# 011235813/cm3

Measured on AMD Instinct MI355X. Metric: env-steps/s (all agents, whole node), higher is better.
Workload: dtype f32; 1 GPU; config_particle_stage2_antipodal.json: 4 agents, 4096 vectorised envs per GPU, max_steps=33, auto-reset, trajectory mode (every tick writes slot t+1 of a [330+1, E, ...] device trajectory incl. termin; envs_per_gpu=4096, n_agents=4, global_envs=4096, mode=trajectory, live_state=True, ticks_per_launch=1, parallelism=env-sharded x1, no data-path collective

## Files before the change

### cm3_amd/csrc/particle.hip

```cpp
#include "common.h"
#include "philox.h"
#include "thresholds.h"

#ifdef CM3_PARTICLE_ILP_TU
#define CM3_PARTICLE_TU 1
#else
#define CM3_PARTICLE_TU 0
#endif

namespace cm3 {

struct ParticleParams;
int particle_ilp_launch_pairs_f32(const ParticleParams &p, int n_agents, int waves_per_wg, hipStream_t stream);
int particle_ilp_launch_agents_f32(const ParticleParams &p, int n_agents, int waves_per_wg, hipStream_t stream);
[[maybe_unused]] constexpr size_t kIlpMaxWaves = 16384;

struct ParticleParams {
  int E;
  int max_steps;
  uint32_t flags;
  int _pad;
  int E0, EN;
  int64_t env_id_base;
  uint64_t seed;
// ... 418 lines not shown
#pragma unroll 1
  for (int t = 0; t < n_ticks; ++t) {
    int act[N];
    int32_t *actions_t = tick_ptr(p.actions, p.st_actions, t);
    if (gen) {
#pragma unroll
      for (int i = 0; i < N; ++i) act[i] = rand5(action_word(ablock[i], episode, (uint32_t)steps));
      if (active) store_row<int32_t, N>(actions_t, e, act);
    } else {
      load_row<int32_t, N>(actions_t, ec, act);
    }

    R fx[N], fy[N];
#pragma unroll
    for (int i = 0; i < N; ++i) {
      R ux = R(0), uy = R(0);
      if (act[i] == 1) ux = R(-1);
      if (act[i] == 2) ux = R(+1);
      if (act[i] == 3) uy = R(-1);
      if (act[i] == 4) uy = R(+1);
      fx[i] = ux * R(5.0) + R(0.0);
      fy[i] = uy * R(5.0) + R(0.0);
    }

#pragma unroll
    for (int a = 0; a < N; ++a) {
#pragma unroll
      for (int b = a + 1; b < N; ++b) {
        R f_x, f_y;
        contact_force<R>(s[a].z - s[b].z, s[a].w - s[b].w, f_x, f_y);
        fx[a] = f_x + fx[a];
        fy[a] = f_y + fy[a];
        fx[b] = (-f_x) + fx[b];
        fy[b] = (-f_y) + fy[b];
      }
    }

#pragma unroll
    for (int i = 0; i < N; ++i) {
      s[i].x = s[i].x * kKeep;
      s[i].y = s[i].y * kKeep;
      s[i].x = s[i].x + (fx[i] / R(1.0)) * kDt;
      s[i].y = s[i].y + (fy[i] / R(1.0)) * kDt;
      s[i].z = s[i].z + s[i].x * kDt;
      s[i].w = s[i].w + s[i].y * kDt;
    }
    steps += 1;
    CM3_STAMP(2, false);

    R rew[N];
    bool all_reached = true;
#pragma unroll
    for (int i = 0; i < N; ++i) {
      const R dx = s[i].z - g[i].x, dy = s[i].w - g[i].y;
      const R d2 = dx * dx + dy * dy;
      rew[i] = R(0) - Math<R>::sqrt(d2);
      all_reached = all_reached && (d2 < Thresh<R>::kReach2);
    }
#pragma unroll
    for (int a = 0; a < N; ++a) {
#pragma unroll
      for (int b = a + 1; b < N; ++b) {
        if (is_collision<R>(s[b].z - s[a].z, s[b].w - s[a].w)) {
          rew[a] = rew[a] - R(1);
          rew[b] = rew[b] - R(1);
          collisions += 2;
        }
      }
    }
    const R reward = sum_agents<R, N>(rew);
    const bool done = (steps == p.max_steps) || all_reached;

    CM3_STAMP(3, false);
    if (active) {
      store_row<R, N>(reinterpret_cast<R *>(tick_ptr(p.reward_n, p.st_reward_n, t)), e, rew);
      reinterpret_cast<R *>(tick_ptr(p.reward, p.st_reward, t))[e] = reward;
      tick_ptr(p.done, p.st_done, t)[e] = done ? 1 : 0;
      if (p.collisions_tick) tick_ptr(p.collisions_tick, p.st_coll, t)[e] = collisions;
    }
    CM3_STAMP(8, false);

    bool was_reset = false;
    if (auto_reset && done) {
      if (active) {
        void *term_state = tick_ptr(p.term_state, p.st_term_state, t);
        void *term_obs = tick_ptr(p.term_obs_others, p.st_term_obs, t);
        if (term_state) {
          V4 *t4 = reinterpret_cast<V4 *>(term_state);
#pragma unroll
          for (int i = 0; i < N; ++i) t4[(size_t)i * E + e] = s[i];
        }
        if (term_obs) store_obs_others_direct<R, N>(s, e, reinterpret_cast<R *>(term_obs));
      }
      episode += 1;
      init_episode<R, N, true>(p, genv, episode, s, g, preset_table(0));
      steps = 0;
      collisions = 0;
      was_reset = true;
    }
    CM3_STAMP(9, false);

    if (active) {
      V4 *sout4 = reinterpret_cast<V4 *>(tick_ptr(p.state_out, p.st_state, t));
#pragma unroll
      for (int i = 0; i < N; ++i) sout4[(size_t)i * E + e] = s[i];
      if (p.goals_out != p.goals_in || was_reset) {
        V2 *gout2 = reinterpret_cast<V2 *>(tick_ptr(p.goals_out, p.st_goals, t));
#pragma unroll
        for (int i = 0; i < N; ++i) gout2[(size_t)i * E + e] = g[i];
      }
      if (p.state_copy) {
#pragma unroll
        for (int i = 0; i < N; ++i) store_obs_vec<SP>(reinterpret_cast<V4 *>(p.state_copy) + ((size_t)i * E + e), s[i]);
      }
      if (was_reset && p.goals_copy) {
#pragma unroll
        for (int i = 0; i < N; ++i) reinterpret_cast<V2 *>(p.goals_copy)[(size_t)i * E + e] = g[i];
      }
    }

    CM3_STAMP(4, false);
    store_obs_others_staged<R, N, SP>(s, &lds_all[wave][0], lane, e0, p.EN,
                                      reinterpret_cast<R *>(tick_ptr(p.obs_others, p.st_obs, t)));
    CM3_STAMP(5, false);
  }

  if (active) {
    int2 m;
    m.x = steps;
    m.y = collisions;
    reinterpret_cast<int2 *>(p.meta_out)[e] = m;
    if (episode != episode_in) p.episode[e] = (int32_t)episode;
  }
  CM3_STAMP(6, true);
  CM3_SPAN_OUT(p.span);
}




template <int N> struct PairGeom {
  static constexpr int NO = N - 1;
  static constexpr int SLOTS = N * NO;
  static constexpr int LA = (N >= 3 && N <= 5) ? (N == 3 ? 2 : 4) : NO;
  static constexpr int pow2ceil(int v) {
    int r = 1;
    while (r < v) r <<= 1;
    return r;
  }
  static constexpr int G = pow2ceil(N * LA);
  static constexpr int EPW = 64 / G;
};

template <typename R, int N, int WAVES, bool FUSED, int SP = kSpPlain, bool LIVE = false, int TU = CM3_PARTICLE_TU>
__global__ void __launch_bounds__(WAVES * 64)
    k_particle_step_pairs(const void *h_state_in, const void *h_goals_in, const int32_t *h_meta_in, const int32_t *h_episode,
                          const int h_E, const uint32_t h_flags, const int h_E0, const int h_EN, const int h_max_steps,
                          const int32_t *h_actions, const ParticleParams p) {
  static_assert(N >= 2, "the pair mapping needs at least two agents");
  using V4 = typename Vec<R>::v4;
  using V2 = typename Vec<R>::v2;
  using PG = PairGeom<N>;
  constexpr int NO = PG::NO, SLOTS = PG::SLOTS, G = PG::G, EPW = PG::EPW, LA = PG::LA;
  static_assert(PairGeom<N>::pow2ceil(SLOTS) == G, "the padded lane layout must not change the group size");
  CM3_SPAN_IN();

  const int lane = threadIdx.x & 63, wave_all = threadIdx.x >> 6;
  const int wave = wave_all;
  const int gslot = lane & (G - 1), sub = lane / G, base = lane - gslot;
  const uint32_t E = (uint32_t)h_E, EN = (uint32_t)h_EN;
  const uint32_t e = (uint32_t)h_E0 + (cm3_xcd_block(h_flags) * WAVES + wave) * EPW + sub;
  const bool env_ok = e < EN;
  const uint32_t ec = env_ok ? e : EN - 1;
  const int i_raw = gslot / LA, k_raw = gslot - i_raw * LA;
  const bool slot_ok = i_raw < N && k_raw < NO;
  const int i = slot_ok ? i_raw : 0, k = slot_ok ? k_raw : 0, j = k < i ? k : k + 1;
  const int vslot = i * NO + k;
  const bool lead = slot_ok && k == 0;
  const bool head = gslot == 0;

  CM3_STAMP(0, false);
  const uint32_t row_i = (uint32_t)i * E, row_j = (uint32_t)j * E;
  V4 si = *at32<const V4>(h_state_in, (row_i + ec) * (uint32_t)sizeof(V4));
  V4 sj = *at32<const V4>(h_state_in, (row_j + ec) * (uint32_t)sizeof(V4));
  V2 gl = *at32<const V2>(h_goals_in, (row_i + ec) * (uint32_t)sizeof(V2));
  const int2 meta = *at32<const int2>(h_meta_in, ec * 8u);
  int steps = meta.x, collisions = meta.y;
  const bool auto_reset = (h_flags & CM3_FLAG_AUTO_RESET) != 0;
  const bool gen = (h_flags & CM3_FLAG_GEN_ACTIONS) != 0;
  uint32_t episode = 0;
  if (gen || (h_flags & CM3_FLAG_AUTO_RESET)) episode = (uint32_t)*at32<const int32_t>(h_episode, ec * 4u);
  const uint32_t episode_in = episode;
  CM3_FETCH_EARLY(p.state_out, p.goals_out, p.goals_in, p.collisions_tick, p.reward_n, p.reward, p.done, p.obs_others, p.meta_out);
  if constexpr (LIVE) CM3_FETCH_EARLY(p.state_copy, p.goals_copy);
  const uint64_t genv = (uint64_t)(p.env_id_base + (int64_t)ec);
  uint32_t aword = 0;
  if (gen) aword = pick_word(action_block(p.seed, genv, (uint32_t)(i >> 2)), i & 3);
  const R kDt = R(0.1), kKeep = R(1 - 0.25);

  CM3_STAMP(1, true);
  CM3_SPAN_MARK(0, true);
  const int n_ticks = FUSED ? p.n_ticks : 1;
#pragma unroll 1
  for (int t = 0; t < n_ticks; ++t) {
    int32_t *actions_t = tick_ptr(p.actions, p.st_actions, t);
    int act = 0;
    R f_x, f_y;
    if (gen) {
      act = rand5(action_word(aword, episode, (uint32_t)steps));
    } else {
      act = *at32<const int32_t>(actions_t, (ec * N + i) * 4u);
    }

    CM3_STAMP(2, false);
    CM3_SPAN_MARK(1, false);
    R ux = R(0), uy = R(0);
    if (act == 1) ux = R(-1);
    if (act == 2) ux = R(+1);
    if (act == 3) uy = R(-1);
    if (act == 4) uy = R(+1);
    R Fx = ux * R(5.0) + R(0.0), Fy = uy * R(5.0) + R(0.0);
    contact_force<R>(si.z - sj.z, si.w - sj.w, f_x, f_y);
    CM3_STAMP(3, false);
    if constexpr (sizeof(R) == 4 && LA == 4 && NO >= 3) {
      Fx = dpp_f32<0x00>(f_x) + Fx;
      Fy = dpp_f32<0x00>(f_y) + Fy;
      Fx = dpp_f32<0x55>(f_x) + Fx;
      Fy = dpp_f32<0x55>(f_y) + Fy;
      Fx = dpp_f32<0xAA>(f_x) + Fx;
      Fy = dpp_f32<0xAA>(f_y) + Fy;
      if constexpr (NO == 4) {
        Fx = dpp_f32<0xFF>(f_x) + Fx;
        Fy = dpp_f32<0xFF>(f_y) + Fy;
      }
    } else if constexpr (N == 2) {
      Fx = f_x + Fx;
      Fy = f_y + Fy;
    } else if constexpr (sizeof(R) == 4 && LA == 2) {
      Fx = dpp_f32<0xA0>(f_x) + Fx;
      Fy = dpp_f32<0xA0>(f_y) + Fy;
      Fx = dpp_f32<0xF5>(f_x) + Fx;
      Fy = dpp_f32<0xF5>(f_y) + Fy;
    } else {
#pragma unroll
      for (int kk = 0; kk < NO; ++kk) {
        const int src = base + i * LA + kk;
        Fx = __shfl(f_x, src, 64) + Fx;
        Fy = __shfl(f_y, src, 64) + Fy;
      }
    }

    si.x = si.x * kKeep;
    si.y = si.y * kKeep;
    si.x = si.x + (Fx / R(1.0)) * kDt;
    si.y = si.y + (Fy / R(1.0)) * kDt;
    si.z = si.z + si.x * kDt;
    si.w = si.w + si.y * kDt;
    steps += 1;
    if constexpr (N == 2 && sizeof(R) == 4) {
      sj.x = dpp_f32<kDppXor1>(si.x);
      sj.y = dpp_f32<kDppXor1>(si.y);
      sj.z = dpp_f32<kDppXor1>(si.z);
      sj.w = dpp_f32<kDppXor1>(si.w);
    } else {
      const int src = base + j * LA;
      sj.x = __shfl(si.x, src, 64);
      sj.y = __shfl(si.y, src, 64);
      sj.z = __shfl(si.z, src, 64);
      sj.w = __shfl(si.w, src, 64);
    }

    CM3_STAMP(4, true);
    CM3_SPAN_MARK(2, false);
    R rew;
    bool reached;
    {
      const R dx = si.z - gl.x, dy = si.w - gl.y;
      const R d2 = dx * dx + dy * dy;
      rew = R(0) - Math<R>::sqrt(d2);
      reached = d2 < Thresh<R>::kReach2;
    }
    const bool hit = slot_ok && is_collision<R>(sj.z - si.z, sj.w - si.w);
    const unsigned long long hits = __ballot(hit);
    const unsigned long long grp = (G == 64) ? hits : ((hits >> base) & ((1ull << (G & 63)) - 1ull));
    const int c_i = __popcll((grp >> (i * LA)) & ((1ull << NO) - 1ull));
#pragma unroll
    for (int c = 0; c < NO; ++c)
      if (c < c_i) rew = rew - R(1);
    collisions += __popcll(grp);
    const unsigned long long rb = __ballot(reached && lead);
    const unsigned long long rgrp = (G == 64) ? rb : ((rb >> base) & ((1ull << (G & 63)) - 1ull));
    const bool all_reached = __popcll(rgrp) == N;
    R rews[N];
    if constexpr (N == 2 && sizeof(R) == 4) {
      rews[0] = dpp_f32<0xA0>(rew);
      rews[1] = dpp_f32<0xF5>(rew);
    } else if constexpr (N == 4 && sizeof(R) == 4) {
      rews[0] = dpp_f32<kDppBcast + 0 * LA>(rew);
      rews[1] = dpp_f32<kDppBcast + 1 * LA>(rew);
      rews[2] = dpp_f32<kDppBcast + 2 * LA>(rew);
      rews[3] = dpp_f32<kDppBcast + 3 * LA>(rew);
    } else {
#pragma unroll
      for (int a = 0; a < N; ++a) rews[a] = __shfl(rew, base + a * LA, 64);
    }
    const R reward = sum_agents<R, N>(rews);
    const bool done = (steps == h_max_steps) || all_reached;

    const int collisions_tick = collisions;

    CM3_STAMP(5, true);
    CM3_SPAN_MARK(3, false);
    bool was_reset = false;
    if (auto_reset && done) {
      if (env_ok) {
        void *term_state = tick_ptr(p.term_state, p.st_term_state, t);
        void *term_obs = tick_ptr(p.term_obs_others, p.st_term_obs, t);
        if (term_state && lead) *at32<V4>(term_state, (row_i + e) * (uint32_t)sizeof(V4)) = si;
        if (term_obs && slot_ok) *at32<V4>(term_obs, (e * SLOTS + vslot) * (uint32_t)sizeof(V4)) = sub4<R, V4>(sj, si);
      }
      episode += 1;
      const uint64_t rseed = reset_seed(p);
      const bool rnd = episode_is_random(p, genv, episode, rseed);
      V2 gj;
      init_agent<R, N, true>(p, genv, episode, rnd, i, si, gl, preset_table(), &rseed);
      init_agent<R, N, true>(p, genv, episode, rnd, j, sj, gj, preset_table(), &rseed);
      steps = 0;
      collisions = 0;
      was_reset = true;
    }

    CM3_STAMP(6, false);
    if (env_ok) {
      if (lead) {
        if (gen) *at32<int32_t>(actions_t, (e * N + i) * 4u) = act;
        *at32<R>(tick_ptr(p.reward_n, p.st_reward_n, t), (e * N + i) * (uint32_t)sizeof(R)) = rew;
        *at32<V4>(tick_ptr(p.state_out, p.st_state, t), (row_i + e) * (uint32_t)sizeof(V4)) = si;
        if (p.goals_out != p.goals_in || was_reset)
          *at32<V2>(tick_ptr(p.goals_out, p.st_goals, t), (row_i + e) * (uint32_t)sizeof(V2)) = gl;
        if constexpr (LIVE)
          store_obs_vec<SP>(at32<V4>(p.state_copy, (row_i + e) * (uint32_t)sizeof(V4)), si);
        if constexpr (!FUSED) {
          if (was_reset && p.goals_copy) *at32<V2>(p.goals_copy, (row_i + e) * (uint32_t)sizeof(V2)) = gl;
        }
      }
      if (slot_ok)
        store_obs_vec<SP>(at32<V4>(tick_ptr(p.obs_others, p.st_obs, t), (e * SLOTS + vslot) * (uint32_t)sizeof(V4)), sub4<R, V4>(sj, si));
      if (head) {
        *at32<R>(tick_ptr(p.reward, p.st_reward, t), e * (uint32_t)sizeof(R)) = reward;
        *at32<uint8_t>(tick_ptr(p.done, p.st_done, t), e) = done ? 1 : 0;
        if (p.collisions_tick) *at32<int32_t>(tick_ptr(p.collisions_tick, p.st_coll, t), e * 4u) = collisions_tick;
        if constexpr (!FUSED) {
          int2 m;
          m.x = steps;
          m.y = collisions;
          *at32<int2>(p.meta_out, e * 8u) = m;
          if (episode != episode_in) *at32<int32_t>(p.episode, e * 4u) = (int32_t)episode;
        }
      }
    }
  }

  CM3_SPAN_MARK(4, false);
  CM3_STAMP(7, false);
  if constexpr (FUSED) {
    if (env_ok && head) {
      int2 m;
      m.x = steps;
      m.y = collisions;
      *at32<int2>(p.meta_out, e * 8u) = m;
      if (episode != episode_in) *at32<int32_t>(p.episode, e * 4u) = (int32_t)episode;
    }
  }
  CM3_STAMP(8, true);
  CM3_SPAN_OUT(p.span);
}

template <int N> struct AgentGeom {
  static constexpr int NO = N - 1;
  static constexpr int G = PairGeom<N>::pow2ceil(N);
  static constexpr int EPW = 64 / G;
  static constexpr int VPE = N * NO;
};

template <typename R, int N, int WAVES, bool FUSED, int SP = kSpPlain, bool LIVE = false, int TU = CM3_PARTICLE_TU>
__global__ void __launch_bounds__(WAVES * 64)
    k_particle_step_agents(const void *h_state_in, const void *h_goals_in, const int32_t *h_meta_in, const int32_t *h_episode,
                           const int h_E, const uint32_t h_flags, const int h_E0, const int h_EN, const int h_max_steps,
                           const int32_t *h_actions, const ParticleParams p) {
  static_assert(N >= 2, "the agent mapping needs at least two agents");
  using V4 = typename Vec<R>::v4;
  using V2 = typename Vec<R>::v2;
  using AG = AgentGeom<N>;
  constexpr int NO = AG::NO, G = AG::G, EPW = AG::EPW, VPE = AG::VPE;
  __shared__ __attribute__((aligned(32))) R lds_all[WAVES][EPW * VPE * 4];
  CM3_SPAN_IN();

  const int lane = threadIdx.x & 63, wave = threadIdx.x >> 6;
  const int gi = lane & (G - 1), sub = lane / G, base = lane - gi;
  const uint32_t E = (uint32_t)h_E, EN = (uint32_t)h_EN;
  const uint32_t e0 = (uint32_t)h_E0 + (cm3_xcd_block(h_flags) * WAVES + wave) * EPW;
  const uint32_t e = e0 + sub;
  const bool env_ok = e < EN;
  const uint32_t ec = env_ok ? e : EN - 1;
  const bool agent_ok = gi < N;
  const int i = agent_ok ? gi : 0;
  const bool mine = env_ok && agent_ok;
  const bool head = env_ok && gi == 0;
  V4 *lds4 = reinterpret_cast<V4 *>(&lds_all[wave][0]);

  CM3_STAMP(0, false);
  const uint32_t row_i = (uint32_t)i * E;
  V4 si = *at32<const V4>(h_state_in, (row_i + ec) * (uint32_t)sizeof(V4));
  V2 gl = *at32<const V2>(h_goals_in, (row_i + ec) * (uint32_t)sizeof(V2));
  const int2 meta = *at32<const int2>(h_meta_in, ec * 8u);
  int steps = meta.x, collisions = meta.y;
  const bool auto_reset = (h_flags & CM3_FLAG_AUTO_RESET) != 0;
  const bool gen = (h_flags & CM3_FLAG_GEN_ACTIONS) != 0;
  uint32_t episode = 0;
  if (gen || (h_flags & CM3_FLAG_AUTO_RESET)) episode = (uint32_t)*at32<const int32_t>(h_episode, ec * 4u);
  const uint32_t episode_in = episode;
  CM3_FETCH_EARLY(p.state_out, p.goals_out, p.goals_in, p.collisions_tick, p.reward_n, p.reward, p.done, p.obs_others, p.meta_out);
  if constexpr (LIVE) CM3_FETCH_EARLY(p.state_copy, p.goals_copy);
  const uint64_t genv = (uint64_t)(p.env_id_base + (int64_t)ec);
  uint32_t aword = 0;
  if (gen) aword = pick_word(action_block(p.seed, genv, (uint32_t)(i >> 2)), i & 3);
  const R kDt = R(0.1), kKeep = R(1 - 0.25);

  long envs_here = (long)EN - (long)e0;
  envs_here = envs_here < 0 ? 0 : (envs_here > EPW ? EPW : envs_here);
  const int nvec = (int)envs_here * VPE;

  auto fill_tile = [&](const V4 (&oj)[N]) {
    if (agent_ok) {
#pragma unroll
      for (int k = 0; k < NO; ++k) {
        const bool below = k < i;
        V4 o;
        o.x = below ? oj[k].x : oj[k + 1].x;
        o.y = below ? oj[k].y : oj[k + 1].y;
        o.z = below ? oj[k].z : oj[k + 1].z;
        o.w = below ? oj[k].w : oj[k + 1].w;
        lds4[sub * VPE + i * NO + k] = sub4<R, V4>(o, si);
      }
    }
    wave_lds_sync();
  };
  auto store_obs = [&](const V4 (&oj)[N], void *dst) {
    fill_tile(oj);
    constexpr int STEPS = (EPW * VPE + 63) / 64;
    V4 row[STEPS];
#pragma unroll
    for (int q = 0; q < STEPS; ++q) row[q] = lds4[(q * 64 + lane) < EPW * VPE ? q * 64 + lane : 0];
#pragma unroll
    for (int q = 0; q < STEPS; ++q) {
      const int f = q * 64 + lane;
      if (f < nvec) store_obs_vec<SP>(at32<V4>(dst, (e0 * VPE + f) * (uint32_t)sizeof(V4)), row[q]);
    }
    wave_lds_sync();
  };

  CM3_STAMP(1, true);
  CM3_SPAN_MARK(0, true);
  const int n_ticks = FUSED ? p.n_ticks : 1;
#pragma unroll 1
  for (int t = 0; t < n_ticks; ++t) {
    int32_t *actions_t = tick_ptr(p.actions, p.st_actions, t);
    int act;
    if (gen) {
      act = rand5(action_word(aword, episode, (uint32_t)steps));
      if (mine) store_small<SP>(at32<int32_t>(actions_t, (e * N + i) * 4u), act);
    } else {
      act = *at32<const int32_t>(actions_t, (ec * N + i) * 4u);
    }

    CM3_STAMP(2, false);
    CM3_SPAN_MARK(1, false);
    R ux = R(0), uy = R(0);
    if (act == 1) ux = R(-1);
    if (act == 2) ux = R(+1);
    if (act == 3) uy = R(-1);
    if (act == 4) uy = R(+1);
    R Fx = ux * R(5.0) + R(0.0), Fy = uy * R(5.0) + R(0.0);
    R dxs[N], dys[N], d2s[N];
    unsigned near_mask = 0;
#pragma unroll
// ... 440 lines not shown
      reinterpret_cast<int2 *>(p.meta_out)[e] = m;
    }
  } else {
#pragma unroll
    for (int i = 0; i < N; ++i) s[i] = sout4[(size_t)i * E + ec];
  }
  store_obs_others_staged<R, N>(s, &lds_all[wave][0], lane, e0, p.EN, reinterpret_cast<R *>(p.obs_others));
}

template <typename R, int N, int WAVES>
__global__ void __launch_bounds__(WAVES * 64) k_particle_observe(const ParticleParams p) {
  using V4 = typename Vec<R>::v4;
  using G = ObsGeom<R, N>;
  __shared__ __attribute__((aligned(32))) R lds_all[WAVES][G::LDS_REALS];
  const int lane = threadIdx.x & 63, wave = threadIdx.x >> 6;
  const size_t e0 = (size_t)p.E0 + ((size_t)blockIdx.x * WAVES + wave) * 64;
  const size_t e = e0 + lane;
  const size_t ec = e < (size_t)p.EN ? e : (size_t)p.EN - 1;
  V4 s[N];
  const V4 *sin4 = reinterpret_cast<const V4 *>(p.state_in);
#pragma unroll
  for (int i = 0; i < N; ++i) s[i] = sin4[(size_t)i * p.E + ec];
  store_obs_others_staged<R, N>(s, &lds_all[wave][0], lane, e0, p.EN, reinterpret_cast<R *>(p.obs_others));
}

enum ParticleOp { kStep = 0, kReset = 1, kObserve = 2 };

static int fill_params(const cm3_particle_desc *d, const cm3_particle_bufs *b, ParticleOp op, const uint8_t *mask,
                       ParticleParams &p) {
  CM3_REQUIRE(d && b, "null desc/bufs");
  CM3_REQUIRE(d->n_envs > 0, "n_envs must be positive (got %d)", d->n_envs);
  CM3_REQUIRE(d->n_agents >= 1 && d->n_agents <= CM3_MAX_AGENTS, "n_agents must be in 1..%d (got %d)",
              CM3_MAX_AGENTS, d->n_agents);
  CM3_REQUIRE(d->max_steps >= 1, "max_steps must be >= 1");
  CM3_REQUIRE((d->flags & ~(CM3_FLAG_AUTO_RESET | CM3_FLAG_GEN_ACTIONS | CM3_FLAG_KERNEL_LANE_PER_ENV |
                            CM3_FLAG_KERNEL_LANE_PER_PAIR | CM3_FLAG_KERNEL_LANE_PER_AGENT | CM3_FLAG_FUSED_TICKS)) == 0,
              "unknown flag bits 0x%x", d->flags);
  {
    const uint32_t k = d->flags & (CM3_FLAG_KERNEL_LANE_PER_ENV | CM3_FLAG_KERNEL_LANE_PER_PAIR | CM3_FLAG_KERNEL_LANE_PER_AGENT);
    CM3_REQUIRE((k & (k - 1)) == 0, "more than one kernel-mapping flag set");
  }
  CM3_REQUIRE(!((d->flags & (CM3_FLAG_KERNEL_LANE_PER_PAIR | CM3_FLAG_KERNEL_LANE_PER_AGENT)) && d->n_agents < 2),
              "the lane-per-pair / lane-per-agent kernels need n_agents >= 2");
  CM3_REQUIRE(b->obs_others, "obs_others is required");
  if (op == kStep) {
    CM3_REQUIRE(b->state_in && b->state_out && b->goals_in && b->goals_out && b->meta_in && b->meta_out,
                "step: state/goals/meta pointers are required");
    CM3_REQUIRE(b->actions && b->reward_n && b->reward && b->done, "step: actions/reward_n/reward/done are required");
    if (d->flags & (CM3_FLAG_AUTO_RESET | CM3_FLAG_GEN_ACTIONS))
      CM3_REQUIRE(b->episode, "episode counter is required with AUTO_RESET / GEN_ACTIONS");
  } else if (op == kReset) {
    CM3_REQUIRE(b->state_out && b->goals_out && b->meta_out && b->episode, "reset: state_out/goals_out/meta_out/episode");
  } else {
    CM3_REQUIRE(b->state_in, "observe: state_in is required");
  }
  CM3_REQUIRE(d->env_offset >= 0 && d->env_count >= 0 && (int64_t)d->env_offset + d->env_count <= d->n_envs &&
                  (d->env_count > 0 || d->env_offset == 0),
              "env_offset / env_count must select a range inside [0, n_envs) (got %d / %d of %d)", d->env_offset,
              d->env_count, d->n_envs);
  memset(&p, 0, sizeof(p));
  p.n_ticks = 1;
  p.E = d->n_envs;
  p.E0 = d->env_offset;
  p.EN = d->env_count > 0 ? d->env_offset + d->env_count : d->n_envs;
  p.max_steps = d->max_steps;
  p.flags = d->flags & ~CM3_FLAG_FUSED_TICKS;
  p.env_id_base = d->env_id_base;
  p.seed = d->seed;
  p.prob_random = d->prob_random;
  p.initial_std = d->initial_std;
  for (int i = 0; i < CM3_MAX_AGENTS; ++i) {
    p.ax[i] = d->agents_x[i];
    p.ay[i] = d->agents_y[i];
    p.lx[i] = d->landmarks_x[i];
    p.ly[i] = d->landmarks_y[i];
  }
  p.state_in = b->state_in;
  p.state_out = b->state_out;
  p.goals_in = b->goals_in;
  p.goals_out = b->goals_out;
  p.meta_in = b->meta_in;
  p.meta_out = b->meta_out;
  p.episode = b->episode;
  p.actions = b->actions;
  p.obs_others = b->obs_others;
  p.reward_n = b->reward_n;
  p.reward = b->reward;
  p.done = b->done;
  p.term_state = b->term_state;
  p.term_obs_others = b->term_obs_others;
  p.collisions_tick = b->collisions_tick;
  p.state_copy = p.goals_copy = nullptr;
  p.reset_mask = mask;
  if (op == kStep) CM3_SPAN_SET(p);
  return CM3_OK;
}

template <typename R, int N, int WAVES>
static int launch_one(const ParticleParams &p, ParticleOp op, hipStream_t stream) {
  const unsigned per_block = WAVES * 64;
  const unsigned blocks = (unsigned)(((size_t)(p.EN - p.E0) + per_block - 1) / per_block);
  switch (op) {
    case kStep: {
      constexpr int kNt = sizeof(R) == 4 ? kSpNt : kSpPlain, kWt = sizeof(R) == 4 ? kSpWt : kSpPlain;
      const bool nt = sizeof(R) == 4 && (p.flags & kFlagObsStoreNt);
      const bool wt = sizeof(R) == 4 && (size_t)(p.EN - p.E0) * ObsGeom<R, N>::REC * sizeof(R) >= kWtMinObsBytes && !p.state_copy;
      note_variant("k_particle_step", (int)sizeof(R), N, WAVES, p.n_ticks > 1,
                   p.n_ticks > 1 ? (nt ? kNt : kSpPlain) : (wt ? kWt : (nt ? kNt : kSpPlain)), 0, CM3_PARTICLE_TU);
      if (p.n_ticks > 1) {
        if (nt) hipLaunchKernelGGL((k_particle_step<R, N, WAVES, true, kNt>), dim3(blocks), dim3(per_block), 0, stream, p);
        else hipLaunchKernelGGL((k_particle_step<R, N, WAVES, true>), dim3(blocks), dim3(per_block), 0, stream, p);
      } else {
        if (wt) hipLaunchKernelGGL((k_particle_step<R, N, WAVES, false, kWt>), dim3(blocks), dim3(per_block), 0, stream, p);
        else if (nt) hipLaunchKernelGGL((k_particle_step<R, N, WAVES, false, kNt>), dim3(blocks), dim3(per_block), 0, stream, p);
        else hipLaunchKernelGGL((k_particle_step<R, N, WAVES, false>), dim3(blocks), dim3(per_block), 0, stream, p);
      }
      break;
    }
    case kReset:
      note_variant("k_particle_reset", (int)sizeof(R), N, WAVES, 0, kSpPlain, 0, CM3_PARTICLE_TU);
      hipLaunchKernelGGL((k_particle_reset<R, N, WAVES>), dim3(blocks), dim3(per_block), 0, stream, p);
      break;
    case kObserve:
      note_variant("k_particle_observe", (int)sizeof(R), N, WAVES, 0, kSpPlain, 0, CM3_PARTICLE_TU);
      hipLaunchKernelGGL((k_particle_observe<R, N, WAVES>), dim3(blocks), dim3(per_block), 0, stream, p);
      break;
  }
  CM3_HIP_CHECK(hipGetLastError());
  return CM3_OK;
}

template <typename R, int N, int WAVES> static int launch_pairs(const ParticleParams &p, hipStream_t stream) {
  if constexpr (N >= 2 && N <= 8) {
    const size_t envs_per_block = (size_t)WAVES * PairGeom<N>::EPW;
    const unsigned raw_blocks = (unsigned)(((size_t)(p.EN - p.E0) + envs_per_block - 1) / envs_per_block);
    const unsigned blocks = cm3_xcd_grid(raw_blocks);
    const uint32_t xf = cm3_xcd_flags(raw_blocks);
    constexpr int kF32 = sizeof(R) == 4 ? kSpNt : kSpPlain;
    const bool nt = sizeof(R) == 4 && (p.flags & kFlagObsStoreNt);
#define CM3_LAUNCH_PAIRS(...)                                                                                               \
  hipLaunchKernelGGL((k_particle_step_pairs<R, N, WAVES, __VA_ARGS__>), dim3(blocks), dim3(WAVES * 64), 0, stream,          \
                     p.state_in, p.goals_in, p.meta_in, (const int32_t *)p.episode, p.E, p.flags | xf, p.E0, p.EN, p.max_steps,   \
                     (const int32_t *)p.actions, p)
    if ((size_t)p.E * PairGeom<N>::SLOTS * 4 * sizeof(R) >= ((size_t)1 << 32))
      return fail(CM3_ERR_INVALID, "the lane-per-pair kernel addresses at most 4 GiB per array: %d envs x %d agents is too large "
                  "(use the default kernel choice)", p.E, N);
    const bool live = p.state_copy != nullptr;
    note_variant("k_particle_step_pairs", (int)sizeof(R), N, WAVES, p.n_ticks > 1, nt ? kF32 : kSpPlain, p.n_ticks == 1 && live,
                 CM3_PARTICLE_TU);
    if (p.n_ticks > 1) {
      if (nt) CM3_LAUNCH_PAIRS(true, kF32);
      else CM3_LAUNCH_PAIRS(true, kSpPlain);
    } else if (live) {
      if (nt) CM3_LAUNCH_PAIRS(false, kF32, true);
      else CM3_LAUNCH_PAIRS(false, kSpPlain, true);
    } else {
      if (nt) CM3_LAUNCH_PAIRS(false, kF32);
      else CM3_LAUNCH_PAIRS(false, kSpPlain);
    }
#undef CM3_LAUNCH_PAIRS
    CM3_HIP_CHECK(hipGetLastError());
    return CM3_OK;
  } else {
    return fail(CM3_ERR_INVALID, "the lane-per-pair kernel needs n_agents in 2..8");
  }
}

constexpr size_t kPairsMaxEnvs = (size_t)1 << 14;

template <typename R, int N, int WAVES> static int launch_agents(const ParticleParams &p, hipStream_t stream) {
  if constexpr (N >= 2) {
    const size_t envs_per_block = (size_t)WAVES * AgentGeom<N>::EPW;
    const unsigned raw_blocks = (unsigned)(((size_t)(p.EN - p.E0) + envs_per_block - 1) / envs_per_block);
    const unsigned blocks = cm3_xcd_grid(raw_blocks);
    const uint32_t xf = cm3_xcd_flags(raw_blocks);
    const bool nt = sizeof(R) == 4 && (p.flags & kFlagObsStoreNt);
#define CM3_LAUNCH_AGENTS(...)                                                                                              \
  hipLaunchKernelGGL((k_particle_step_agents<R, N, WAVES, __VA_ARGS__>), dim3(blocks), dim3(WAVES * 64), 0, stream,         \
                     p.state_in, p.goals_in, p.meta_in, (const int32_t *)p.episode, p.E, p.flags | xf, p.E0, p.EN, p.max_steps,   \
                     (const int32_t *)p.actions, p)
    if ((size_t)p.E * AgentGeom<N>::VPE * 4 * sizeof(R) >= ((size_t)1 << 32))
      return fail(CM3_ERR_INVALID, "the lane-per-agent kernel addresses at most 4 GiB per array: %d envs x %d agents is too large", p.E, N);
    const bool live = p.state_copy != nullptr;
    constexpr int kNt = sizeof(R) == 4 ? kSpNt : kSpPlain, kWt = sizeof(R) == 4 ? kSpWt : kSpPlain;
    const bool wt = sizeof(R) == 4 && (size_t)(p.EN - p.E0) * AgentGeom<N>::VPE * 4 * sizeof(R) >= kWtMinObsBytes;
    if constexpr (N == 8 && sizeof(R) == 4) {
      if (p.n_ticks == 1 && (size_t)(p.EN - p.E0) <= kAgents2MaxEnvs) {
        const unsigned raw2 = (unsigned)(((size_t)(p.EN - p.E0) + (size_t)WAVES * 4 - 1) / ((size_t)WAVES * 4));
        const unsigned blocks2 = cm3_xcd_grid(raw2);
        const uint32_t xf2 = cm3_xcd_flags(raw2);
#define CM3_LAUNCH_AGENTS2(...)                                                                                             \
  hipLaunchKernelGGL((k_particle_step_agents2<WAVES, __VA_ARGS__>), dim3(blocks2), dim3(WAVES * 64), 0, stream, p.state_in,  \
                     p.goals_in, p.meta_in, (const int32_t *)p.episode, p.E, p.flags | xf2, p.E0, p.EN, p.max_steps,         \
                     (const int32_t *)p.actions, p)
        const bool early = wt && (size_t)(p.EN - p.E0) <= kAgents2EarlyMaxEnvs;
        note_variant("k_particle_step_agents2", 4, 8, WAVES, 0, wt ? kWt : (nt ? kNt : kSpPlain), live, CM3_PARTICLE_TU, early);
        if (live) {
          if (early) CM3_LAUNCH_AGENTS2(kWt, true, true);
          else if (wt) CM3_LAUNCH_AGENTS2(kWt, true);
          else if (nt) CM3_LAUNCH_AGENTS2(kNt, true);
          else CM3_LAUNCH_AGENTS2(kSpPlain, true);
        } else {
          if (early) CM3_LAUNCH_AGENTS2(kWt, false, true);
          else if (wt) CM3_LAUNCH_AGENTS2(kWt);
          else if (nt) CM3_LAUNCH_AGENTS2(kNt);
          else CM3_LAUNCH_AGENTS2(kSpPlain);
        }
#undef CM3_LAUNCH_AGENTS2
        CM3_HIP_CHECK(hipGetLastError());
        return CM3_OK;
      }
    }
    note_variant("k_particle_step_agents", (int)sizeof(R), N, WAVES, p.n_ticks > 1,
                 p.n_ticks > 1 ? (nt ? kNt : kSpPlain) : (wt ? kWt : (nt ? kNt : kSpPlain)), p.n_ticks == 1 && live, CM3_PARTICLE_TU);
    if (p.n_ticks > 1) {
      if (nt) CM3_LAUNCH_AGENTS(true, kNt);
      else CM3_LAUNCH_AGENTS(true, kSpPlain);
    } else if (live) {
      if (wt) CM3_LAUNCH_AGENTS(false, kWt, true);
      else if (nt) CM3_LAUNCH_AGENTS(false, kNt, true);
      else CM3_LAUNCH_AGENTS(false, kSpPlain, true);
    } else {
      if (wt) CM3_LAUNCH_AGENTS(false, kWt);
      else if (nt) CM3_LAUNCH_AGENTS(false, kNt);
      else CM3_LAUNCH_AGENTS(false, kSpPlain);
    }
#undef CM3_LAUNCH_AGENTS
    CM3_HIP_CHECK(hipGetLastError());
    return CM3_OK;
  } else {
    return fail(CM3_ERR_INVALID, "the lane-per-agent kernel needs n_agents >= 2");
  }
}

constexpr int kSharedEnvWaves = 4;
template <typename R, int N> static int launch_n(const ParticleParams &p, ParticleOp op, hipStream_t stream) {
  if (op == kStep) {
    constexpr size_t kInf = ~(size_t)0;
    constexpr size_t kPairMax = N > 8 ? 0 : (N == 2 ? 32768 : (N == 3 ? 24576 : (N == 4 ? 12288 : kPairsMaxEnvs)));
    constexpr size_t kAgentLo = N == 4 ? 12289 : (N == 5 ? 10240 : (N == 6 ? 8192 : (N == 7 ? 6144 : (N == 8 ? 4096 : (N > 8 ? 1024 : kInf)))));
    constexpr size_t kAgentHi = N == 4 || N == 5 ? 40960 : (N == 6 ? 1572864 : (N >= 7 ? 786432 : 0));
    bool pairs = N >= 2 && (size_t)p.E <= kPairMax;
    bool agents = N >= 4 && (size_t)p.E >= kAgentLo && (size_t)p.E <= kAgentHi;
    if ((size_t)p.E * N * (N - 1) * 4 * sizeof(R) >= ((size_t)1 << 32)) pairs = agents = false;
    if (p.flags & CM3_FLAG_KERNEL_LANE_PER_ENV) pairs = agents = false;
    if (p.flags & CM3_FLAG_KERNEL_LANE_PER_PAIR) { pairs = true; agents = false; }
    if (N > 8 && pairs) return fail(CM3_ERR_INVALID, "the lane-per-pair kernel needs n_agents in 2..8");
    if (p.flags & CM3_FLAG_KERNEL_LANE_PER_AGENT) agents = true;
    if (agents) {
      const size_t waves = ((size_t)p.E + AgentGeom<(N >= 2 ? N : 2)>::EPW - 1) / AgentGeom<(N >= 2 ? N : 2)>::EPW;
#ifndef CM3_PARTICLE_ILP_TU
      if constexpr (sizeof(R) == 4 && N >= 2)
        if (waves <= kIlpMaxWaves) return particle_ilp_launch_agents_f32(p, N, waves < 256 ? 1 : kSharedEnvWaves, stream);
#endif
      if (waves < 256) return launch_agents<R, N, 1>(p, stream);
      return launch_agents<R, N, kSharedEnvWaves>(p, stream);
    }
    if (pairs) {
      constexpr int NP = (N >= 2 && N <= 8) ? N : 2;
      const size_t waves = ((size_t)p.E + PairGeom<NP>::EPW - 1) / PairGeom<NP>::EPW;
#ifndef CM3_PARTICLE_ILP_TU
      if constexpr (sizeof(R) == 4 && N >= 2)
        if (waves <= kIlpMaxWaves) return particle_ilp_launch_pairs_f32(p, N, waves < 256 ? 1 : kSharedEnvWaves, stream);
#endif
      if (waves < 256) return launch_pairs<R, N, 1>(p, stream);
      return launch_pairs<R, N, kSharedEnvWaves>(p, stream);
    }
  }
  if ((size_t)p.E <= (size_t)128 * 1024) return launch_one<R, N, 1>(p, op, stream);
  return launch_one<R, N, 4>(p, op, stream);
}

template <typename R> static int launch(const ParticleParams &p, int n_agents, ParticleOp op, hipStream_t stream) {
  switch (n_agents) {
    case 1: return launch_n<R, 1>(p, op, stream);
    case 2: return launch_n<R, 2>(p, op, stream);
    case 3: return launch_n<R, 3>(p, op, stream);
    case 4: return launch_n<R, 4>(p, op, stream);
    case 5: return launch_n<R, 5>(p, op, stream);
    case 6: return launch_n<R, 6>(p, op, stream);
    case 7: return launch_n<R, 7>(p, op, stream);
    case 8: return launch_n<R, 8>(p, op, stream);
    case 9: return launch_n<R, 9>(p, op, stream);
    case 10: return launch_n<R, 10>(p, op, stream);
  }
  return fail(CM3_ERR_INVALID, "n_agents %d unsupported", n_agents);
}

template <typename R>
static int particle_call(const cm3_particle_desc *d, const cm3_particle_bufs *b, ParticleOp op, const uint8_t *mask,
                         void *stream) {
  ParticleParams p;
  int rc = fill_params(d, b, op, mask, p);
  if (rc != CM3_OK) return rc;
  return launch<R>(p, d->n_agents, op, (hipStream_t)stream);
}

static uint32_t obs_store_nt(size_t obs_stride, int n_ticks) {
  return obs_stride * (size_t)n_ticks >= ((size_t)128 << 20) ? kFlagObsStoreNt : 0u;
}

template <typename R>
static int particle_rollout(const cm3_particle_desc *d, const cm3_particle_traj *t, int32_t n_ticks, void *stream) {
  CM3_REQUIRE(d && t, "null desc/traj");
  CM3_REQUIRE(n_ticks >= 1, "n_ticks must be >= 1");
  CM3_REQUIRE(t->state && t->goals && t->obs_others && t->actions && t->reward_n && t->reward && t->done && t->meta,
// ... 158 lines not shown
```

Measured before the change: 1.710 billion env-steps/s.

## Add specialised N=4 live-rollout pair kernel with cheaper cross-lane and store paths

Adds a FIX template variant of the pair kernel, chosen for the f32, N=4, 4-wave, live-state, auto-reset, generated-actions case with non-temporal obs stores. It fixes the runtime flags and pointer checks at compile time and uses umul24 for the row offsets. Neighbour state is gathered with ds_bpermute instead of __shfl. The collision penalty and the reached test use fixed-mask ballots plus DPP broadcasts instead of the per-slot popcount loop. Stores skip tick_ptr and pass addresses through an opaque asm barrier, and goals and episode are written on reset. The variant is narrow and duplicates logic, so it can drift from the generic path.

```diff
diff --git a/cm3_amd/csrc/particle.hip b/cm3_amd/csrc/particle.hip
--- a/cm3_amd/csrc/particle.hip
+++ b/cm3_amd/csrc/particle.hip
@@ -594,7 +594,24 @@
   static constexpr int EPW = 64 / G;
 };
 
-template <typename R, int N, int WAVES, bool FUSED, int SP = kSpPlain, bool LIVE = false, int TU = CM3_PARTICLE_TU>
+__device__ __forceinline__ float from_lane(float v, int src) {
+  return __int_as_float(__builtin_amdgcn_ds_bpermute(src << 2, __float_as_int(v)));
+}
+__device__ __forceinline__ double from_lane(double v, int src) {
+  const int2 w = *reinterpret_cast<const int2 *>(&v);
+  int2 r;
+  r.x = __builtin_amdgcn_ds_bpermute(src << 2, w.x);
+  r.y = __builtin_amdgcn_ds_bpermute(src << 2, w.y);
+  return *reinterpret_cast<const double *>(&r);
+}
+
+constexpr int kFixLiveRollout = 1;
+__device__ __forceinline__ uint32_t opq(uint32_t v) {
+  asm volatile("" : "+v"(v));
+  return v;
+}
+
+template <typename R, int N, int WAVES, bool FUSED, int SP = kSpPlain, bool LIVE = false, int TU = CM3_PARTICLE_TU, int FIX = 0>
 __global__ void __launch_bounds__(WAVES * 64)
     k_particle_step_pairs(const void *h_state_in, const void *h_goals_in, const int32_t *h_meta_in, const int32_t *h_episode,
                           const int h_E, const uint32_t h_flags, const int h_E0, const int h_EN, const int h_max_steps,
@@ -605,6 +622,9 @@
   using PG = PairGeom<N>;
   constexpr int NO = PG::NO, SLOTS = PG::SLOTS, G = PG::G, EPW = PG::EPW, LA = PG::LA;
   static_assert(PairGeom<N>::pow2ceil(SLOTS) == G, "the padded lane layout must not change the group size");
+  static_assert(FIX == 0 || (LIVE && !FUSED && N == 4 && WAVES == 4 && sizeof(R) == 4),
+                "the fixed variant is the per-tick live-state rollout at N = 4 (C2)");
+  constexpr bool kFix = FIX == kFixLiveRollout;
   CM3_SPAN_IN();
 
   const int lane = threadIdx.x & 63, wave_all = threadIdx.x >> 6;
@@ -622,16 +642,16 @@
   const bool head = gslot == 0;
 
   CM3_STAMP(0, false);
-  const uint32_t row_i = (uint32_t)i * E, row_j = (uint32_t)j * E;
+  const uint32_t row_i = kFix ? __umul24((uint32_t)i, E) : (uint32_t)i * E, row_j = kFix ? __umul24((uint32_t)j, E) : (uint32_t)j * E;
   V4 si = *at32<const V4>(h_state_in, (row_i + ec) * (uint32_t)sizeof(V4));
   V4 sj = *at32<const V4>(h_state_in, (row_j + ec) * (uint32_t)sizeof(V4));
   V2 gl = *at32<const V2>(h_goals_in, (row_i + ec) * (uint32_t)sizeof(V2));
   const int2 meta = *at32<const int2>(h_meta_in, ec * 8u);
   int steps = meta.x, collisions = meta.y;
-  const bool auto_reset = (h_flags & CM3_FLAG_AUTO_RESET) != 0;
-  const bool gen = (h_flags & CM3_FLAG_GEN_ACTIONS) != 0;
+  const bool auto_reset = kFix || (h_flags & CM3_FLAG_AUTO_RESET) != 0;
+  const bool gen = kFix || (h_flags & CM3_FLAG_GEN_ACTIONS) != 0;
   uint32_t episode = 0;
-  if (gen || (h_flags & CM3_FLAG_AUTO_RESET)) episode = (uint32_t)*at32<const int32_t>(h_episode, ec * 4u);
+  if (gen || auto_reset) episode = (uint32_t)*at32<const int32_t>(h_episode, ec * 4u);
   const uint32_t episode_in = episode;
   CM3_FETCH_EARLY(p.state_out, p.goals_out, p.goals_in, p.collisions_tick, p.reward_n, p.reward, p.done, p.obs_others, p.meta_out);
   if constexpr (LIVE) CM3_FETCH_EARLY(p.state_copy, p.goals_copy);
@@ -706,10 +726,10 @@
       sj.w = dpp_f32<kDppXor1>(si.w);
     } else {
       const int src = base + j * LA;
-      sj.x = __shfl(si.x, src, 64);
-      sj.y = __shfl(si.y, src, 64);
-      sj.z = __shfl(si.z, src, 64);
-      sj.w = __shfl(si.w, src, 64);
+      sj.x = from_lane(si.x, src);
+      sj.y = from_lane(si.y, src);
+      sj.z = from_lane(si.z, src);
+      sj.w = from_lane(si.w, src);
     }
 
     CM3_STAMP(4, true);
@@ -722,17 +742,30 @@
       rew = R(0) - Math<R>::sqrt(d2);
       reached = d2 < Thresh<R>::kReach2;
     }
-    const bool hit = slot_ok && is_collision<R>(sj.z - si.z, sj.w - si.w);
-    const unsigned long long hits = __ballot(hit);
-    const unsigned long long grp = (G == 64) ? hits : ((hits >> base) & ((1ull << (G & 63)) - 1ull));
-    const int c_i = __popcll((grp >> (i * LA)) & ((1ull << NO) - 1ull));
-#pragma unroll
-    for (int c = 0; c < NO; ++c)
-      if (c < c_i) rew = rew - R(1);
-    collisions += __popcll(grp);
-    const unsigned long long rb = __ballot(reached && lead);
-    const unsigned long long rgrp = (G == 64) ? rb : ((rb >> base) & ((1ull << (G & 63)) - 1ull));
-    const bool all_reached = __popcll(rgrp) == N;
+    const bool near = is_collision<R>(sj.z - si.z, sj.w - si.w);
+    const bool hit = slot_ok && near;
+    bool all_reached;
+    if constexpr (kFix) {
+      const unsigned long long hits = __ballot(near) & 0x7777777777777777ull, rb = __ballot(reached) & 0x1111111111111111ull;
+      const R hf = hit ? R(1) : R(0);
+      asm("" : "+v"(rew));
+      rew = rew - dpp_f32<0x00>(hf);
+      rew = rew - dpp_f32<0x55>(hf);
+      rew = rew - dpp_f32<0xAA>(hf);
+      collisions += __popc((uint32_t)(hits >> base) & 0xFFFFu);
+      all_reached = ((uint32_t)(rb >> base) & 0xFFFFu) == 0x1111u;
+    } else {
+      const unsigned long long hits = __ballot(hit);
+      const unsigned long long rb = __ballot(reached && lead);
+      const unsigned long long grp = (G == 64) ? hits : ((hits >> base) & ((1ull << (G & 63)) - 1ull));
+      const int c_i = __popcll((grp >> (i * LA)) & ((1ull << NO) - 1ull));
+#pragma unroll
+      for (int c = 0; c < NO; ++c)
+        if (c < c_i) rew = rew - R(1);
+      collisions += __popcll(grp);
+      const unsigned long long rgrp = (G == 64) ? rb : ((rb >> base) & ((1ull << (G & 63)) - 1ull));
+      all_reached = __popcll(rgrp) == N;
+    }
     R rews[N];
     if constexpr (N == 2 && sizeof(R) == 4) {
       rews[0] = dpp_f32<0xA0>(rew);
@@ -758,8 +791,8 @@
       if (env_ok) {
         void *term_state = tick_ptr(p.term_state, p.st_term_state, t);
         void *term_obs = tick_ptr(p.term_obs_others, p.st_term_obs, t);
-        if (term_state && lead) *at32<V4>(term_state, (row_i + e) * (uint32_t)sizeof(V4)) = si;
-        if (term_obs && slot_ok) *at32<V4>(term_obs, (e * SLOTS + vslot) * (uint32_t)sizeof(V4)) = sub4<R, V4>(sj, si);
+        if ((kFix || term_state) && lead) *at32<V4>(term_state, (row_i + e) * (uint32_t)sizeof(V4)) = si;
+        if ((kFix || term_obs) && slot_ok) *at32<V4>(term_obs, (e * SLOTS + vslot) * (uint32_t)sizeof(V4)) = sub4<R, V4>(sj, si);
       }
       episode += 1;
       const uint64_t rseed = reset_seed(p);
@@ -770,10 +803,36 @@
       steps = 0;
       collisions = 0;
       was_reset = true;
+      if constexpr (kFix) {
+        if (env_ok && lead) {
+          *at32<V2>(p.goals_out, opq((row_i + e) * (uint32_t)sizeof(V2))) = gl;
+          *at32<V2>(p.goals_copy, opq((row_i + e) * (uint32_t)sizeof(V2))) = gl;
+        }
+        if (env_ok && head) *at32<int32_t>(p.episode, opq(e * 4u)) = (int32_t)episode;
+      }
     }
 
     CM3_STAMP(6, false);
-    if (env_ok) {
+    if constexpr (kFix) {
+      if (env_ok && slot_ok) {
+        store_obs_vec<SP>(at32<V4>(p.obs_others, opq((e * SLOTS + vslot) * (uint32_t)sizeof(V4))), sub4<R, V4>(sj, si));
+        if (lead) {
+          store_obs_vec<SP>(at32<V4>(p.state_copy, opq((row_i + e) * (uint32_t)sizeof(V4))), si);
+          *at32<V4>(p.state_out, opq((row_i + e) * (uint32_t)sizeof(V4))) = si;
+          *at32<int32_t>(p.actions, opq((e * N + i) * 4u)) = act;
+          *at32<R>(p.reward_n, opq((e * N + i) * (uint32_t)sizeof(R))) = rew;
+          if (head) {
+            *at32<R>(p.reward, opq(e * (uint32_t)sizeof(R))) = reward;
+            *at32<uint8_t>(p.done, opq(e)) = done ? 1 : 0;
+            *at32<int32_t>(p.collisions_tick, opq(e * 4u)) = collisions_tick;
+            int2 m;
+            m.x = steps;
+            m.y = collisions;
+            *at32<int2>(p.meta_out, opq(e * 8u)) = m;
+          }
+        }
+      }
+    } else if (env_ok) {
       if (lead) {
         if (gen) *at32<int32_t>(actions_t, (e * N + i) * 4u) = act;
         *at32<R>(tick_ptr(p.reward_n, p.st_reward_n, t), (e * N + i) * (uint32_t)sizeof(R)) = rew;
@@ -1520,6 +1579,14 @@
       if (nt) CM3_LAUNCH_PAIRS(true, kF32);
       else CM3_LAUNCH_PAIRS(true, kSpPlain);
     } else if (live) {
+      const bool fixed = (p.flags & CM3_FLAG_GEN_ACTIONS) && (p.flags & CM3_FLAG_AUTO_RESET) && p.goals_out == p.goals_in &&
+                         p.goals_copy && p.collisions_tick && p.term_state && p.term_obs_others;
+      if constexpr (sizeof(R) == 4 && CM3_PARTICLE_TU == 1 && N == 4 && WAVES == 4)
+        if (nt && fixed) {
+          CM3_LAUNCH_PAIRS(false, kF32, true, CM3_PARTICLE_TU, kFixLiveRollout);
+          CM3_HIP_CHECK(hipGetLastError());
+          return CM3_OK;
+        }
       if (nt) CM3_LAUNCH_PAIRS(false, kF32, true);
       else CM3_LAUNCH_PAIRS(false, kSpPlain, true);
     } else {
```

Result: faster. 1.761 billion env-steps/s (median of 6 runs) (+2.9%).
